# 4paradigm/OpenEmbedding

Measured on AMD Instinct MI355X. Metric: samples/sec DeepFM Criteo, higher is better.
Workload: dtype bf16; 1 GPU; model=deepfm-dim9, global_batch=4096, fields=26, dense_features=13, optimizer=adagrad, graph=True, prefetch=False, table=array, cache_mb=0, parallelism=single-gpu

## Files before the change

### openembedding_amd/ops/csrc/bindings.cpp

```cpp

#include <torch/extension.h>
#include <ATen/cuda/CUDAContext.h>
#include <c10/cuda/CUDAGuard.h>

#include <cstdint>
#include <tuple>
#include <vector>

typedef unsigned long long u64;
typedef int64_t i64;
typedef struct ihipStream_t* hipStream_t_;

extern "C" {
void emb_unique(const i64*, long, u64*, int*, long, int*, unsigned char*,
                i64*, i64*, int*, const i64*, int, hipStream_t_);
void emb_ht_lookup(u64*, int*, long, const i64*, long, int*, i64*, i64*,
                   unsigned char*, int, const int*, long, hipStream_t_);
void emb_ht_rehash(const u64*, const int*, long, u64*, int*, long,
                   hipStream_t_);
void emb_array_touch(unsigned char*, const i64*, long, long, long, i64*,
                     unsigned char*, const int*, hipStream_t_);
void emb_gather_init(float*, float*, long, long, const i64*,
                     const unsigned char*, const i64*, long, const i64*,
                     float*, int, float, float, float, u64, const float*,
                     const int*, hipStream_t_);
void emb_reduce_by_inverse(const i64*, const float*, long, long, float*, u64*,
                           long, hipStream_t_);
void emb_reduce_bags_by_inverse(const i64*, const float*, long, long,
                                const int*, const i64*, long, int, float*,
                                u64*, long, hipStream_t_);
void emb_pool_fwd(const float*, long, long, const i64*, long, const void*,
                  int, long, const i64*, long, int, float*, int*,
                  hipStream_t_);
void emb_pool_fwd_weighted(const float*, long, long, const i64*, long,
                           const void*, int, long, const i64*, long, int,
                           const float*, float*, int*, float*, hipStream_t_);
void emb_reduce_bags_weighted_by_inverse(const i64*, const float*, long, long,
                                         const int*, const float*,
// ... 77 lines not shown
using OptTensor = c10::optional<torch::Tensor>;

hipStream_t_ cur_stream() {
    return reinterpret_cast<hipStream_t_>(
        at::cuda::getCurrentCUDAStream().stream());
}

long next_pow2(long x) {
    long p = 16;
    while (p < x) p <<= 1;
    return p;
}

const int* u_ptr(const OptTensor& u_dev) {
    if (!u_dev.has_value()) return nullptr;
    TORCH_CHECK(u_dev->dtype() == torch::kInt32, "u_dev must be int32");
    return u_dev->data_ptr<int>();
}

#define CHECK_GPU(t) TORCH_CHECK((t).is_cuda(), #t " must be on GPU")
#define CHECK_CONT(t) TORCH_CHECK((t).is_contiguous(), #t " must be contiguous")


std::tuple<torch::Tensor, torch::Tensor, torch::Tensor> unique_bounded(
    torch::Tensor keys, OptTensor field_offsets) {
    CHECK_GPU(keys); CHECK_CONT(keys);
    TORCH_CHECK(keys.dtype() == torch::kInt64);
    const i64* foff = nullptr;
    int F = 0;
    if (field_offsets.has_value() && field_offsets->numel()) {
        CHECK_GPU(*field_offsets); CHECK_CONT(*field_offsets);
        TORCH_CHECK(field_offsets->dtype() == torch::kInt64,
                    "field_offsets must be int64");
        TORCH_CHECK(keys.numel() % field_offsets->numel() == 0,
                    "keys length must be a multiple of field_offsets");
        foff = field_offsets->data_ptr<i64>();
        F = (int)field_offsets->numel();
    }
    const c10::cuda::CUDAGuard guard(keys.device());
    long n = keys.numel();
    auto opts_i64 = keys.options();
    auto opts_i32 = keys.options().dtype(torch::kInt32);
    auto opts_u8 = keys.options().dtype(torch::kUInt8);
    long cap = next_pow2(2 * n);
    auto tk = torch::empty({cap}, opts_i64);
    auto tv = torch::empty({cap}, opts_i32);
    auto slot_of = torch::empty({n}, opts_i32);
    auto is_first = torch::empty({n}, opts_u8);
    auto uk = torch::empty({n}, opts_i64);
    auto inverse = torch::empty({n}, opts_i64);
    auto counter = torch::empty({1}, opts_i32);
    emb_unique(keys.data_ptr<i64>(), n, (u64*)tk.data_ptr<i64>(),
               tv.data_ptr<int>(), cap, slot_of.data_ptr<int>(),
               is_first.data_ptr<uint8_t>(), uk.data_ptr<i64>(),
               inverse.data_ptr<i64>(), counter.data_ptr<int>(), foff, F,
               cur_stream());
    return {uk, inverse, counter};
}

std::tuple<torch::Tensor, torch::Tensor> unique_inverse(torch::Tensor keys) {
    auto r = unique_bounded(keys, c10::nullopt);
    long u = std::get<2>(r).item<int>();
    return {std::get<0>(r).narrow(0, 0, u), std::get<1>(r)};
}


std::tuple<torch::Tensor, torch::Tensor> ht_lookup(
    torch::Tensor tk, torch::Tensor tv, torch::Tensor keys,
    torch::Tensor nrows, torch::Tensor slot_keys, bool insert,
    OptTensor u_dev) {
    CHECK_GPU(keys); CHECK_CONT(keys);
    const c10::cuda::CUDAGuard guard(keys.device());
    long n = keys.numel();
    auto slots = torch::empty({n}, keys.options());
    auto new_mask = torch::empty({n}, keys.options().dtype(torch::kUInt8));
    if (n)
        emb_ht_lookup((u64*)tk.data_ptr<i64>(), tv.data_ptr<int>(),
                      tk.numel(), keys.data_ptr<i64>(), n,
                      nrows.data_ptr<int>(), slot_keys.data_ptr<i64>(),
                      slots.data_ptr<i64>(), new_mask.data_ptr<uint8_t>(),
// ... 54 lines not shown
                    keys.data_ptr<i64>(), n,
                    inverse.has_value() ? inverse->data_ptr<i64>() : nullptr,
                    out_ptr, (int)init_cat,
                    (float)p0, (float)p1, (float)p2, (u64)seed,
                    sd ? state_init_row.data_ptr<float>() : nullptr,
                    u_ptr(u_dev), cur_stream());
    return out;
}


std::tuple<torch::Tensor, torch::Tensor> reduce_by_inverse(
    torch::Tensor inverse, torch::Tensor grads, int64_t u) {
    CHECK_GPU(grads); CHECK_CONT(grads);
    TORCH_CHECK(grads.dtype() == torch::kFloat32,
                "reduce_by_inverse: grads must be float32");
    const c10::cuda::CUDAGuard guard(grads.device());
    long n = grads.size(0);
    long dim = grads.size(1);
    auto ugrads = torch::empty({u, dim}, grads.options());
    auto counts = torch::empty({u}, grads.options().dtype(torch::kInt64));
    emb_reduce_by_inverse(inverse.data_ptr<i64>(), grads.data_ptr<float>(), n,
                          dim, ugrads.data_ptr<float>(),
                          (u64*)counts.data_ptr<i64>(), u, cur_stream());
    return {ugrads, counts};
}


std::tuple<torch::Tensor, torch::Tensor> pool_fwd(
    torch::Tensor rows, OptTensor inverse, OptTensor map,
    torch::Tensor offsets, int64_t mode, bool want_bag_of) {
    CHECK_GPU(rows); CHECK_CONT(rows);
    CHECK_GPU(offsets); CHECK_CONT(offsets);
    TORCH_CHECK(rows.dtype() == torch::kFloat32 && rows.dim() == 2,
                "pool_fwd: rows must be float32 [R, dim]");
    TORCH_CHECK(offsets.dtype() == torch::kInt64 && offsets.dim() == 1
                && offsets.numel() >= 1,
                "pool_fwd: offsets must be int64 [B+1]");
    TORCH_CHECK(mode >= 0 && mode <= 2, "pool_fwd: bad mode");
    const void* map_ptr = nullptr;
    int map_kind = 0;
    long u = 0;
    if (map.has_value()) {
        CHECK_GPU(*map); CHECK_CONT(*map);
        u = map->numel();
        if (map->dtype() == torch::kInt64) {
            map_kind = 1;
// ... 846 lines not shown
                 w2t.data_ptr(), w1t.data_ptr(), H, Hp, dz1.data_ptr(),
                 dz2.data_ptr(), dz3.data_ptr(), dx0.data_ptr(), bptr,
                 (int)bm, (int)frag, cur_stream());
    return {dx0, dz1, dz2, dz3};
}

}

PYBIND11_MODULE(TORCH_EXTENSION_NAME, m) {
    m.def("unique_inverse", &unique_inverse, "hash-based unique+inverse");
    m.def("unique_bounded", &unique_bounded,
          "unique+inverse without host sync (n-sized buffer + device "
          "count); optional fused per-field key offsets",
          pybind11::arg("keys"),
          pybind11::arg("field_offsets") = pybind11::none());
    m.def("ht_lookup", &ht_lookup, "hash table lookup/insert");
    m.def("ht_rehash", &ht_rehash, "hash table rehash into larger table");
    m.def("array_touch", &array_touch,
          "array-table slot compute + valid-bitmap touch");
    m.def("gather_init", &gather_init,
          "row gather with fused lazy init (+ optional duplicate scatter)");
    m.def("reduce_by_inverse", &reduce_by_inverse,
          "grad reduce-by-key with counts (LDS-aggregated)");
    m.def("pool_fwd", &pool_fwd,
          "segment-pooled gather (sum/mean/sqrtn) over ragged bags; also "
          "emits each element's bag for the backward",
          pybind11::arg("rows"), pybind11::arg("inverse"),
          pybind11::arg("map"), pybind11::arg("offsets"),
          pybind11::arg("mode"), pybind11::arg("want_bag_of") = true);
    m.def("reduce_bags_by_inverse", &reduce_bags_by_inverse,
          "grad reduce-by-key reading the pooled [B, dim] gradient through "
          "bag_of (no [nnz, dim] expansion)");
    m.def("pool_fwd_weighted", &pool_fwd_weighted,
          "pool_fwd with per-sample weights; also emits bag_of and the "
          "per-bag combiner scale for the backward",
          pybind11::arg("rows"), pybind11::arg("inverse"),
          pybind11::arg("map"), pybind11::arg("offsets"),
          pybind11::arg("weights"), pybind11::arg("mode"),
          pybind11::arg("out") = pybind11::none(),
          pybind11::arg("bag_scale") = pybind11::none());
    m.def("reduce_bags_weighted_by_inverse",
          &reduce_bags_weighted_by_inverse,
          "bag-indirected grad reduce with the per-element factor "
          "weights[e] * bag_scale[bag_of[e]]");
    m.def("pool_wgrad", &pool_wgrad,
          "gradient of the weighted pool w.r.t. its per-sample weights",
// ... 97 lines not shown
```

### openembedding_amd/ops/csrc/embops.hip

```cpp

#include <hip/hip_runtime.h>
#include <cstdint>

#define DEV static __device__ __forceinline__

typedef unsigned long long u64;
typedef long long i64;

static constexpr u64 EMPTY = ~0ull;
static constexpr int BLOCK = 256;

static inline int cdiv(long a, long b) { return (int)((a + b - 1) / b); }
static inline int grid1d(long n) {
    long g = (n + BLOCK - 1) / BLOCK;
    return (int)(g < 1 ? 1 : g);
}


template <typename T>
__global__ void k_fill(T* __restrict__ p, long n, T v) {
    long i = (long)blockIdx.x * blockDim.x + threadIdx.x;
    if (i < n) p[i] = v;
}

static inline void fill_u64(u64* p, long n, u64 v, hipStream_t s) {
    if (n) k_fill<u64><<<(int)((n + 255) / 256), 256, 0, s>>>(p, n, v);
}
static inline void fill_i32(int* p, long n, int v, hipStream_t s) {
    if (n) k_fill<int><<<(int)((n + 255) / 256), 256, 0, s>>>(p, n, v);
}
static inline void fill_u8(unsigned char* p, long n, unsigned char v,
                           hipStream_t s) {
    if (n) k_fill<unsigned char><<<(int)((n + 255) / 256), 256, 0, s>>>(p, n, v);
}
static inline void fill_f32(float* p, long n, float v, hipStream_t s) {
    if (n) k_fill<float><<<(int)((n + 255) / 256), 256, 0, s>>>(p, n, v);
}

__global__ void k_unique_reset(u64* __restrict__ tk, long cap,
                               unsigned char* __restrict__ is_first, long n,
                               int* __restrict__ counter) {
    long i = (long)blockIdx.x * blockDim.x + threadIdx.x;
    if (i < cap) tk[i] = ~0ull;
    if (i < n) is_first[i] = 0;
    if (i == 0) *counter = 0;
}

__global__ void k_reduce_reset(float* __restrict__ ugrads, long ne,
                               u64* __restrict__ counts, long u) {
    long i = (long)blockIdx.x * blockDim.x + threadIdx.x;
    if (i < ne) ugrads[i] = 0.0f;
    if (i < u) counts[i] = 0ull;
}

__global__ void k_pad_reset(u64* __restrict__ send_keys,
                            int* __restrict__ send_src, long total,
                            int* __restrict__ counts, long world) {
    long i = (long)blockIdx.x * blockDim.x + threadIdx.x;
    if (i < total) { send_keys[i] = ~0ull; send_src[i] = -1; }
    if (i < world) counts[i] = 0;
}


DEV u64 splitmix64(u64 z) {
    z += 0x9E3779B97F4A7C15ull;
    z = (z ^ (z >> 30)) * 0xBF58476D1CE4E5B9ull;
    z = (z ^ (z >> 27)) * 0x94D049BB133111EBull;
    return z ^ (z >> 31);
// ... 17 lines not shown
    float r = sqrtf(-2.0f * logf(1.0f - u1));
    return r * cosf(2.0f * 3.14159265358979323846f * u2);
}

DEV float init_value(int cat, float p0, float p1, float p2,
                     u64 seed, u64 key, u64 col) {
    if (cat == INIT_CONSTANT) return p0;
    if (cat == INIT_UNIFORM) {
        float u = uniform01(seed, key, col, 0);
        return p0 + u * p1;
    }
    float z = normal01(seed, key, col, 0);
    if (p2 > 0.1f) {
        for (int attempt = 1; attempt < 16 && z > p2; ++attempt)
            z = normal01(seed, key, col, attempt);
    }
    return p0 + p1 * z;
}


#define ULDS 1024
#define UA_ITERS 8
#define UI_ILP 4

__global__ void k_unique_insert(const i64* __restrict__ keys, long n,
                                u64* __restrict__ tk, long mask,
                                int* __restrict__ slot_of,
                                unsigned char* __restrict__ is_first,
                                const i64* __restrict__ foff, int F) {
    __shared__ u64 lkeys[ULDS];
    __shared__ int lslot[ULDS];
    for (int t = threadIdx.x; t < ULDS; t += blockDim.x) lkeys[t] = EMPTY;
    __syncthreads();

    long i = (long)blockIdx.x * blockDim.x + threadIdx.x;
    u64 k = 0;
    i64 kin = 0;
    if (i < n) {
        kin = keys[i];
        if (foff) kin += foff[(int)i % F];
    }
    int lh = -1;
    bool lds_winner = false, lds_ok = false;
    if (i < n && (u64)kin == EMPTY) {
        is_first[i] = 1;
        slot_of[i] = -1;
    } else if (i < n) {
        k = (u64)kin;
        u64 hh = splitmix64(k);
        lh = (int)(hh & (ULDS - 1));
        for (int probes = 0; probes < 64; ++probes) {
            u64 cur = atomicCAS(&lkeys[lh], EMPTY, k);
            if (cur == EMPTY) { lds_winner = true; lds_ok = true; break; }
            if (cur == k) { lds_ok = true; break; }
            lh = (lh + 1) & (ULDS - 1);
        }
        if (lds_winner || !lds_ok) {
            u64 h = splitmix64(k) & (u64)mask;
            long found = -1;
            for (long p = 0; p <= mask; ++p) {
                u64 cur = tk[h];
                if (cur == k) { found = (long)h; break; }
                if (cur == EMPTY) {
                    u64 prev = atomicCAS(&tk[h], EMPTY, k);
                    if (prev == EMPTY) {
                        is_first[i] = 1; found = (long)h; break;
                    }
                    if (prev == k) { found = (long)h; break; }
                }
                h = (h + 1) & (u64)mask;
            }
            if (found < 0) is_first[i] = 1;
            slot_of[i] = found >= 0 ? (int)found : -1;
            if (lds_winner)
                lslot[lh] = found >= 0 ? (int)found : (int)(-2 - i);
        }
    }
    __syncthreads();
    if (i < n && lds_ok && !lds_winner) slot_of[i] = lslot[lh];
}

__global__ void k_unique_assign(const i64* __restrict__ keys, long n,
                                const int* __restrict__ slot_of,
                                const unsigned char* __restrict__ is_first,
                                int* __restrict__ tv,
                                i64* __restrict__ unique_keys,
                                int* __restrict__ counter,
                                i64* __restrict__ inverse,
                                const i64* __restrict__ foff, int F) {
    const int lane = threadIdx.x & 63;
    const long stride = (long)gridDim.x * blockDim.x;
    long i0 = (long)blockIdx.x * blockDim.x + threadIdx.x;
    u64 ballots[UA_ITERS];
    int total = 0;
    #pragma unroll
    for (int t = 0; t < UA_ITERS; ++t) {
        long i = i0 + t * stride;
        bool first = (i < n) && is_first[i];
        ballots[t] = __ballot(first);
        total += __popcll(ballots[t]);
    }
    if (!total) return;
    int base = 0;
    if (lane == 0) base = atomicAdd(counter, total);
    base = __shfl(base, 0, 64);
    #pragma unroll
    for (int t = 0; t < UA_ITERS; ++t) {
        u64 b = ballots[t];
        if (b & (1ull << lane)) {
            long i = i0 + t * stride;
            int uid = base + __popcll(b & ((1ull << lane) - 1ull));
            i64 kin = keys[i];
            if (foff) kin += foff[(int)i % F];
            unique_keys[uid] = kin;
            int s = slot_of[i];
            if (s >= 0) tv[s] = uid;
            else inverse[i] = uid;
        }
        base += __popcll(b);
    }
}

__global__ void k_unique_inverse(long n, const int* __restrict__ slot_of,
                                 const int* __restrict__ tv,
                                 i64* __restrict__ inverse) {
    const long stride = (long)gridDim.x * blockDim.x;
    long i0 = (long)blockIdx.x * blockDim.x + threadIdx.x;
    int s[UI_ILP];
    #pragma unroll
    for (int t = 0; t < UI_ILP; ++t) {
        long i = i0 + t * stride;
        s[t] = (i < n) ? slot_of[i] : -1;
    }
    int v[UI_ILP];
    #pragma unroll
    for (int t = 0; t < UI_ILP; ++t)
        v[t] = (s[t] >= 0) ? tv[s[t]] : 0;
    #pragma unroll
    for (int t = 0; t < UI_ILP; ++t) {
        long i = i0 + t * stride;
        if (i >= n) continue;
        if (s[t] >= 0) inverse[i] = (i64)v[t];
        else if (s[t] <= -2) inverse[i] = inverse[-2 - s[t]];
    }
}


__global__ void k_ht_lookup(u64* __restrict__ tk, int* __restrict__ tv,
                            long mask, const i64* __restrict__ keys, long n,
                            int* __restrict__ nrows,
                            i64* __restrict__ slot_keys,
                            i64* __restrict__ slots,
                            unsigned char* __restrict__ new_mask,
                            int insert, const int* __restrict__ u_dev,
                            long row_cap) {
    long i = (long)blockIdx.x * blockDim.x + threadIdx.x;
    if (i >= n) return;
    if (u_dev && i >= *u_dev) {
        slots[i] = -1;
        if (new_mask) new_mask[i] = 0;
        return;
    }
    u64 k = (u64)keys[i];
    if (k == EMPTY) {
// ... 493 lines not shown
        long src;
        if constexpr (WEIGHTED)
            src = reduce_src_w(bag_of[i], B, weights[i], bag_scale, scale);
        else
            src = reduce_src(bag_of[i], n, offsets, B, mode, scale);
        if (src < 0) return;
        atomicAdd(&ugrads[inverse[i] * dim + j],
                  grads[(u64)src * dim + j] * scale);
    } else {
        atomicAdd(&ugrads[inverse[i] * dim + j], grads[e]);
    }
}

template <bool BAG = false>
__global__ void k_reduce_counts(const i64* __restrict__ inverse, long n,
                                u64* __restrict__ counts,
                                const int* __restrict__ bag_of, long B) {
    long i = (long)blockIdx.x * blockDim.x + threadIdx.x;
    if (i >= n) return;
    if (BAG && (bag_of[i] < 0 || bag_of[i] >= B)) return;
    atomicAdd(&counts[inverse[i]], 1ull);
}

#define WG_ILP 4
template <int G, typename MapT>
__global__ void k_pool_wgrad(const float* __restrict__ rows, long R,
                             long dim, const i64* __restrict__ inverse,
                             long nnz, const MapT* __restrict__ map, long u,
                             const float* __restrict__ weights,
                             const int* __restrict__ bag_of,
                             const float* __restrict__ bag_scale,
                             const float* __restrict__ out,
                             const float* __restrict__ grad_out, long B,
                             int mode, float* __restrict__ dw) {
    const long e = ((long)blockIdx.x * blockDim.x + threadIdx.x) / G;
    const int lane = threadIdx.x % G;
    if (e >= nnz) return;
    const int bag = bag_of[e];
    if (bag < 0 || bag >= B) {
        if (lane == 0) dw[e] = 0.0f;
        return;
    }
    const long nidx = map ? u : R;
    const long row = pool_row(e, nnz, inverse, map, nidx, R);
    const float scale = bag_scale[bag];
    const float* __restrict__ g = grad_out + (u64)bag * dim;
// ... 563 lines not shown
    else LAUNCH_POOL(64, 4, 4);
#undef LAUNCH_POOL
}

template <bool WEIGHTED, typename Resolve>
static void pool_lookup_dispatch(const float* rows, long dim, long nnz,
                                 const i64* offsets, long B, int mode,
                                 const float* weights, float* out,
                                 const Resolve& resolve,
                                 hipStream_t stream) {
    if (B == 0) return;
#define LAUNCH_LOOKUP(G, CF, ILP)                                           \
    k_pool_lookup<G, CF, ILP, WEIGHTED, Resolve>                            \
        <<<grid1d(B * G), BLOCK, 0, stream>>>(rows, dim, nnz, offsets, B,   \
                                              mode, weights, out, resolve)
    if (dim <= 16) LAUNCH_LOOKUP(16, 1, 16);
    else if (dim <= 32) LAUNCH_LOOKUP(16, 2, 8);
    else if (dim <= 64) LAUNCH_LOOKUP(64, 1, 16);
    else if (dim <= 128) LAUNCH_LOOKUP(64, 2, 8);
    else LAUNCH_LOOKUP(64, 4, 4);
#undef LAUNCH_LOOKUP
}

extern "C" {

void emb_unique(const i64* keys, long n, u64* tk, int* tv, long cap,
                int* slot_of, unsigned char* is_first, i64* unique_keys,
                i64* inverse, int* counter, const i64* foff, int F,
                hipStream_t stream) {
    {
        long mx = cap > n ? cap : n;
        k_unique_reset<<<(int)((mx + 255) / 256), 256, 0, stream>>>(
            tk, cap, is_first, n, counter);
    }
    long mask = cap - 1;
    k_unique_insert<<<grid1d(n), BLOCK, 0, stream>>>(keys, n, tk, mask,
                                                     slot_of, is_first,
                                                     foff, F);
    int ga = grid1d((n + UA_ITERS - 1) / UA_ITERS);
    int gi = grid1d((n + UI_ILP - 1) / UI_ILP);
    k_unique_assign<<<ga, BLOCK, 0, stream>>>(keys, n, slot_of, is_first,
                                              tv, unique_keys, counter,
                                              inverse, foff, F);
    k_unique_inverse<<<gi, BLOCK, 0, stream>>>(n, slot_of, tv, inverse);
}

void emb_ht_lookup(u64* tk, int* tv, long cap, const i64* keys, long n,
                   int* nrows, i64* slot_keys, i64* slots,
                   unsigned char* new_mask, int insert, const int* u_dev,
                   long row_cap, hipStream_t stream) {
    k_ht_lookup<<<grid1d(n), BLOCK, 0, stream>>>(tk, tv, cap - 1, keys, n,
                                                 nrows, slot_keys, slots,
                                                 new_mask, insert, u_dev,
                                                 row_cap);
}

void emb_ht_rehash(const u64* tk_old, const int* tv_old, long cap_old,
                   u64* tk_new, int* tv_new, long cap_new,
                   hipStream_t stream) {
    fill_u64(tk_new, cap_new, EMPTY, stream);
    k_ht_rehash<<<grid1d(cap_old), BLOCK, 0, stream>>>(
        tk_old, tv_old, cap_old, tk_new, tv_new, cap_new - 1);
}

void emb_array_touch(unsigned char* valid, const i64* keys, long n,
                     long shard_num, long cap, i64* slots,
                     unsigned char* new_mask, const int* u_dev,
// ... 314 lines not shown
```

### openembedding_amd/ops/dispatch.py

```python

from __future__ import annotations

from typing import Tuple

import torch

from . import require_hip


def _use_hip(t: torch.Tensor) -> bool:
    return t.is_cuda



def unique_inverse(keys: torch.Tensor) -> Tuple[torch.Tensor, torch.Tensor]:
    if keys.numel() == 0:
        return keys.clone(), torch.empty(0, dtype=torch.int64, device=keys.device)
    if _use_hip(keys):
        ext = require_hip()
        if ext is not None:
            return ext.unique_inverse(keys)
    return torch.unique(keys, return_inverse=True)



def reduce_by_inverse(inverse: torch.Tensor, grads: torch.Tensor, u: int
                      ) -> Tuple[torch.Tensor, torch.Tensor]:
    if _use_hip(grads) and grads.dtype == torch.float32:
        ext = require_hip()
        if ext is not None:
            return ext.reduce_by_inverse(inverse, grads, u)
    ugrads = torch.zeros((u, grads.shape[1]), dtype=grads.dtype,
                         device=grads.device)
    ugrads.index_add_(0, inverse, grads)
    counts = torch.bincount(inverse, minlength=u).to(torch.int64)
    return ugrads, counts



POOL_MODES = {"sum": 0, "mean": 1, "sqrtn": 2}


def _bag_scale(offsets: torch.Tensor, nnz: int, mode: str,
               dtype: torch.dtype) -> torch.Tensor:
    off = offsets.clamp(0, nnz)
    length = (off[1:] - off[:-1]).clamp(min=0).to(dtype)
    if mode == "sum":
        scale = torch.ones_like(length)
    elif mode == "mean":
        scale = 1.0 / length
    else:
        scale = 1.0 / length.sqrt()
    return torch.where(length > 0, scale, torch.zeros_like(scale))


def _bag_of(offsets: torch.Tensor, nnz: int) -> torch.Tensor:
    off = offsets.clamp(0, nnz)
    pos = torch.arange(nnz, device=offsets.device)
# ... 205 lines not shown
```

### openembedding_amd/parallel/sharded.py

```python

from __future__ import annotations

import dataclasses
import os
from typing import Dict, List, Optional

import torch

from ..core.variable import VariableShard
from ..ops import dispatch as ops
from ..utils.metrics import REGISTRY, stage_timer
from . import comm


class _PaddedPlan:

    def __init__(self, world: int, n: int, device: torch.device):
        slack = float(os.environ.get("OEAMD_A2A_SLACK", "2.0"))
        cap = int(-(-n * slack // world))
        cap = (cap + 255) // 256 * 256
        self.cap = max(1, min(n, cap))
        self.world = world
        total = world * self.cap
        self.send_keys = torch.full((total,), -1, dtype=torch.int64,
                                    device=device)
        self.send_src = torch.full((total,), -1, dtype=torch.int32,
                                   device=device)
        self.pos_of = torch.full((n,), -1, dtype=torch.int32, device=device)
        self.counts = torch.zeros(world, dtype=torch.int32, device=device)
        self.overflow = torch.zeros(1, dtype=torch.int32, device=device)
        self.overflow_host = 0


@dataclasses.dataclass
class PullHandle:

    shape: torch.Size
    unique: Optional[torch.Tensor] = None
    inverse: Optional[torch.Tensor] = None
    order: Optional[torch.Tensor] = None
    send_splits: Optional[List[int]] = None
    recv_splits: Optional[List[int]] = None
    owner_unique: Optional[torch.Tensor] = None
    owner_inverse: Optional[torch.Tensor] = None
    bounded: bool = False
    u_dev: Optional[torch.Tensor] = None
    slots: Optional[torch.Tensor] = None
    owner_u_dev: Optional[torch.Tensor] = None
    owner_slots: Optional[torch.Tensor] = None
    padded: bool = False
    plan: Optional["_PaddedPlan"] = None
    owner_cpu: Optional[tuple] = None
    bag_of: Optional[torch.Tensor] = None
    bag_scale: Optional[torch.Tensor] = None
    pooled_rows: Optional[torch.Tensor] = None


class ShardedVariable:

    def __init__(self, shard: VariableShard, storage=None):
        self.shard = shard
        self.storage = storage
        self.world_size = shard.shard_num
        self.rank = shard.shard_id
        self.stat_pull_indices = 0
        self.stat_pull_unique = 0
        self._plans: Dict[int, Optional[_PaddedPlan]] = {}
        self._commits_since_check = 0


    @property
    def meta(self):
        return self.shard.meta

    @property
    def variable_id(self):
        return self.shard.meta.variable_id

# ... 34 lines not shown
                r = self._pull_remote_padded(indices, flat, field_offsets)
                if r is not None:
                    return r
            if bounded_ok:
                return self._pull_remote_bounded(indices, flat,
                                                 field_offsets)
        unique, inverse = ops.unique_inverse(flat)
        self.stat_pull_unique += unique.numel()
        REGISTRY.add("pull_indices", n)
        REGISTRY.add("pull_unique", unique.numel())
        h = PullHandle(shape=indices.shape, unique=unique, inverse=inverse)
        if self.world_size == 1:
            rows_u = (self.shard.pull_readonly(unique) if readonly
                      else self.shard.pull(unique))
        else:
            rows_u = self._pull_remote(h, readonly)
        out = rows_u.index_select(0, inverse)
        out = out.view(*h.shape, self.shard.dim)
        return out, h

    def _pull_local_bounded(self, indices: torch.Tensor, flat: torch.Tensor,
                            field_offsets: torch.Tensor = None):
        ext = self.shard.ext
        uk_buf, inverse, u_dev = ext.unique_bounded(flat, field_offsets)
        out, slots = self.shard.pull_bounded(uk_buf, u_dev, inverse)
        h = PullHandle(shape=indices.shape, unique=uk_buf, inverse=inverse,
                       bounded=True, u_dev=u_dev, slots=slots)
        return out.view(*indices.shape, self.shard.dim), h

    def pull_pooled(self, values: torch.Tensor, offsets: torch.Tensor,
                    mode: str, readonly: bool = False, pre=None,
                    weights: torch.Tensor = None, wgrad: bool = False):
        flat = values.reshape(-1).to(torch.int64)
        dim = self.shard.dim
        gpu = getattr(self.shard, "pull_bounded", None) is not None
        remote = self.world_size > 1 or self._force_remote
        if gpu and not remote and not readonly and pre is None:
            self.stat_pull_indices += flat.numel()
            ext = self.shard.ext
            uk_buf, inverse, u_dev = ext.unique_bounded(flat, None)
            bag_scale = None
            if weights is None:
                out, slots, bag_of = self.shard.pull_pooled_bounded(
                    uk_buf, u_dev, inverse, offsets, ops.POOL_MODES[mode])
            else:
                out, slots, bag_of, bag_scale = \
                    self.shard.pull_pooled_bounded(
                        uk_buf, u_dev, inverse, offsets,
                        ops.POOL_MODES[mode], weights)
            h = PullHandle(shape=flat.shape, unique=uk_buf, inverse=inverse,
# ... 91 lines not shown
                dev = device if comm.backend() == "nccl" else "cpu"
                t = torch.tensor([n, -n], dtype=torch.int64, device=dev)
                dist.all_reduce(t, op=dist.ReduceOp.MIN)
                if int(t[0]) != n or int(-t[1]) != n:
                    self._plans[n] = None
                    return None
            pair = [_PaddedPlan(self.world_size, n, device),
                    _PaddedPlan(self.world_size, n, device), 0]
            self._plans[n] = pair
        pair[2] ^= 1
        return pair[pair[2]]

    def _pull_remote_padded(self, indices: torch.Tensor,
                            flat: torch.Tensor,
                            field_offsets: torch.Tensor = None):
        world = self.world_size
        dim = self.shard.dim
        dev = flat.device
        n = flat.numel()
        plan = self._get_padded_plan(n, dev)
        if plan is None:
            return None
        gpu = getattr(self.shard, "pull_bounded", None) is not None
        if gpu:
            ext = self.shard.ext
            uk_buf, inverse, u_dev = ext.unique_bounded(flat, field_offsets)
            ext.bucketize_pad(uk_buf, u_dev, world, plan.cap,
                              plan.send_keys, plan.send_src, plan.pos_of,
                              plan.counts, plan.overflow)
        else:
            uk_buf, inverse = ops.unique_inverse(flat)
            u_dev = None
            self._bucketize_pad_torch(uk_buf, plan)
        REGISTRY.add("pull_indices", n)
        REGISTRY.add("pull_wire_keys", plan.send_keys.numel())
        h = PullHandle(shape=indices.shape, unique=uk_buf, inverse=inverse,
                       u_dev=u_dev, padded=True, plan=plan)
        recv_keys = comm.all_to_all_equal(plan.send_keys, world)
        if gpu:
            uk2_buf, inv2, u2_dev = ext.unique_bounded(recv_keys)
            rows_back, slots2 = self.shard.pull_bounded(uk2_buf, u2_dev,
                                                        inv2)
            h.owner_unique = uk2_buf
            h.owner_inverse = inv2
            h.owner_u_dev = u2_dev
            h.owner_slots = slots2
        else:
            rows_back = self._owner_pull_padded_torch(recv_keys, h)
        rows_recv = comm.all_to_all_equal(rows_back, world)
        if gpu:
            out = ext.scatter_out(rows_recv, inverse, plan.pos_of, n)
        else:
            pos = plan.pos_of.index_select(0, inverse).long()
            out = rows_recv.index_select(0, pos.clamp(min=0))
            out = out.masked_fill((pos < 0).unsqueeze(1), 0.0)
        return out.view(*indices.shape, dim), h

    def _bucketize_pad_torch(self, uk: torch.Tensor,
                             plan: _PaddedPlan) -> None:
        world, cap = plan.world, plan.cap
# ... 98 lines not shown
            h.owner_unique = uk2_buf
            h.owner_inverse = inv2
            h.owner_u_dev = u2_dev
            h.owner_slots = slots2
        else:
            uk2, inv2 = ops.unique_inverse(recv_keys)
            rows_u2 = (self.shard.pull_readonly(uk2) if readonly
                       else self.shard.pull(uk2))
            rows_back = rows_u2.index_select(0, inv2)
            h.owner_unique = uk2
            h.owner_inverse = inv2
        rows_sorted = comm.all_to_all_v(rows_back, recv_splits, send_splits)
        rows_u = torch.empty_like(rows_sorted)
        rows_u.index_copy_(0, order, rows_sorted)
        h.order = order
        h.send_splits = send_splits
        h.recv_splits = recv_splits
        return rows_u


    def push(self, h: PullHandle, grads: torch.Tensor) -> None:
        dim = self.shard.dim
        g = grads.reshape(-1, dim)
        ugrads, counts = ops.reduce_by_inverse(h.inverse, g,
                                               h.unique.numel())
        self._apply_reduced(h, ugrads, counts)

    def push_pooled(self, h: PullHandle, grad_out: torch.Tensor,
                    offsets: torch.Tensor, mode: str,
                    weights: torch.Tensor = None, out: torch.Tensor = None,
                    wgrad: bool = False):
        g = grad_out.reshape(-1, self.shard.dim)
        if weights is None:
            ugrads, counts = ops.reduce_bags_by_inverse(
                h.inverse, g, h.bag_of, offsets, mode, h.unique.numel())
            self._apply_reduced(h, ugrads, counts)
            return None
        nnz = h.bag_of.numel()
        w = weights[:nnz].contiguous()
        ugrads, counts = ops.reduce_bags_weighted_by_inverse(
            h.inverse, g, h.bag_of, w, h.bag_scale, h.unique.numel())
        dw = None
        if wgrad:
            if h.pooled_rows is not None:
                dw = ops.pool_wgrad(h.pooled_rows, None, None, w, h.bag_of,
                                    h.bag_scale, out, g, mode)
                h.pooled_rows = None
            else:
# ... 57 lines not shown
```

Baseline: 17.52 million samples/s.

## Build inverted index during unique and reduce gradients by segment without atomics

The unique kernels now also count occurrences per slot, compute per-uid segment offsets with a wave prefix scan, and write a permutation that groups each unique key's occurrences. This gives an inverted index. A new segmented reduce kernel walks each uid's list to sum gradients and set counts, which replaces the atomic reduce-by-inverse in push. Lists longer than a threshold are handled by dedicated blocks. The cost is extra atomics, memory traffic and bookkeeping inside unique, and it is on by default through an environment flag.

```diff
diff --git a/openembedding_amd/ops/csrc/bindings.cpp b/openembedding_amd/ops/csrc/bindings.cpp
--- a/openembedding_amd/ops/csrc/bindings.cpp
+++ b/openembedding_amd/ops/csrc/bindings.cpp
@@ -14,6 +14,15 @@
 extern "C" {
 void emb_unique(const i64*, long, u64*, int*, long, int*, unsigned char*,
                 i64*, i64*, int*, const i64*, int, hipStream_t_);
+void emb_unique_indexed(const i64*, long, u64*, int*, long, int*,
+                        unsigned char*, i64*, i64*, int*, const i64*, int,
+                        int*, int*, int*, int*, int*, int*, int*, long, int*,
+                        int*, hipStream_t_);
+int emb_seg_threshold();
+int emb_seg_max_dim();
+void emb_reduce_by_index(const int*, const int*, const int*, const int*,
+                         const int*, long, const float*, long, long,
+                         const int*, float*, u64*, hipStream_t_);
 void emb_ht_lookup(u64*, int*, long, const i64*, long, int*, i64*, i64*,
                    unsigned char*, int, const int*, long, hipStream_t_);
 void emb_ht_rehash(const u64*, const int*, long, u64*, int*, long,
@@ -137,8 +146,8 @@
 #define CHECK_CONT(t) TORCH_CHECK((t).is_contiguous(), #t " must be contiguous")
 
 
-std::tuple<torch::Tensor, torch::Tensor, torch::Tensor> unique_bounded(
-    torch::Tensor keys, OptTensor field_offsets) {
+std::vector<torch::Tensor> unique_bounded_impl(
+    torch::Tensor keys, OptTensor field_offsets, bool indexed) {
     CHECK_GPU(keys); CHECK_CONT(keys);
     TORCH_CHECK(keys.dtype() == torch::kInt64);
     const i64* foff = nullptr;
@@ -165,12 +174,47 @@
     auto uk = torch::empty({n}, opts_i64);
     auto inverse = torch::empty({n}, opts_i64);
     auto counter = torch::empty({1}, opts_i32);
-    emb_unique(keys.data_ptr<i64>(), n, (u64*)tk.data_ptr<i64>(),
-               tv.data_ptr<int>(), cap, slot_of.data_ptr<int>(),
-               is_first.data_ptr<uint8_t>(), uk.data_ptr<i64>(),
-               inverse.data_ptr<i64>(), counter.data_ptr<int>(), foff, F,
-               cur_stream());
-    return {uk, inverse, counter};
+    if (!indexed) {
+        emb_unique(keys.data_ptr<i64>(), n, (u64*)tk.data_ptr<i64>(),
+                   tv.data_ptr<int>(), cap, slot_of.data_ptr<int>(),
+                   is_first.data_ptr<uint8_t>(), uk.data_ptr<i64>(),
+                   inverse.data_ptr<i64>(), counter.data_ptr<int>(), foff, F,
+                   cur_stream());
+        return {uk, inverse, counter};
+    }
+    TORCH_CHECK(n < (1L << 31), "unique_bounded_indexed: n must fit int32");
+    auto tct = torch::empty({2, cap}, opts_i32);
+    auto segs = torch::empty({4, n}, opts_i32);
+    long long_cap = n / (emb_seg_threshold() + 1) + 1;
+    auto long_list = torch::empty({long_cap}, opts_i32);
+    auto ctr = torch::empty({32}, opts_i32);
+    auto seg_off = segs.select(0, 0), seg_cnt = segs.select(0, 1);
+    auto perm = segs.select(0, 2), rank = segs.select(0, 3);
+    auto n_long = ctr.narrow(0, 16, 1);
+    emb_unique_indexed(keys.data_ptr<i64>(), n, (u64*)tk.data_ptr<i64>(),
+                       tv.data_ptr<int>(), cap, slot_of.data_ptr<int>(),
+                       is_first.data_ptr<uint8_t>(), uk.data_ptr<i64>(),
+                       inverse.data_ptr<i64>(), counter.data_ptr<int>(), foff,
+                       F, tct.data_ptr<int>(), tct.data_ptr<int>() + cap,
+                       rank.data_ptr<int>(), seg_off.data_ptr<int>(),
+                       seg_cnt.data_ptr<int>(), perm.data_ptr<int>(),
+                       long_list.data_ptr<int>(), long_cap,
+                       ctr.data_ptr<int>(), n_long.data_ptr<int>(),
+                       cur_stream());
+    return {uk, inverse, counter, seg_off, seg_cnt, perm, long_list, n_long};
+}
+
+std::tuple<torch::Tensor, torch::Tensor, torch::Tensor> unique_bounded(
+    torch::Tensor keys, OptTensor field_offsets) {
+    auto r = unique_bounded_impl(keys, field_offsets, false);
+    return {r[0], r[1], r[2]};
+}
+
+std::tuple<torch::Tensor, torch::Tensor, torch::Tensor, torch::Tensor,
+           torch::Tensor, torch::Tensor, torch::Tensor, torch::Tensor>
+unique_bounded_indexed(torch::Tensor keys, OptTensor field_offsets) {
+    auto r = unique_bounded_impl(keys, field_offsets, true);
+    return {r[0], r[1], r[2], r[3], r[4], r[5], r[6], r[7]};
 }
 
 std::tuple<torch::Tensor, torch::Tensor> unique_inverse(torch::Tensor keys) {
@@ -271,6 +315,39 @@
     emb_reduce_by_inverse(inverse.data_ptr<i64>(), grads.data_ptr<float>(), n,
                           dim, ugrads.data_ptr<float>(),
                           (u64*)counts.data_ptr<i64>(), u, cur_stream());
+    return {ugrads, counts};
+}
+
+std::tuple<torch::Tensor, torch::Tensor> reduce_by_index(
+    torch::Tensor seg_off, torch::Tensor seg_cnt, torch::Tensor perm,
+    torch::Tensor long_list, torch::Tensor n_long, torch::Tensor grads,
+    torch::Tensor u_dev) {
+    CHECK_GPU(grads); CHECK_CONT(grads);
+    TORCH_CHECK(grads.dtype() == torch::kFloat32 && grads.dim() == 2,
+                "reduce_by_index: grads must be float32 [n, dim]");
+    long n = grads.size(0);
+    long dim = grads.size(1);
+    TORCH_CHECK(dim <= emb_seg_max_dim(),
+                "reduce_by_index: dim above the kernel's ladder");
+    for (const auto* t : {&seg_off, &seg_cnt, &perm, &long_list, &n_long,
+                          &u_dev}) {
+        CHECK_GPU(*t); CHECK_CONT(*t);
+        TORCH_CHECK(t->dtype() == torch::kInt32,
+                    "reduce_by_index: index tensors must be int32");
+    }
+    TORCH_CHECK(seg_off.numel() == n && seg_cnt.numel() == n
+                && perm.numel() == n,
+                "reduce_by_index: index does not match grads");
+    TORCH_CHECK(n_long.numel() == 1 && u_dev.numel() == 1);
+    const c10::cuda::CUDAGuard guard(grads.device());
+    auto ugrads = torch::empty({n, dim}, grads.options());
+    auto counts = torch::empty({n}, grads.options().dtype(torch::kInt64));
+    emb_reduce_by_index(seg_off.data_ptr<int>(), seg_cnt.data_ptr<int>(),
+                        perm.data_ptr<int>(), long_list.data_ptr<int>(),
+                        n_long.data_ptr<int>(), long_list.numel(),
+                        grads.data_ptr<float>(), n, dim,
+                        u_dev.data_ptr<int>(), ugrads.data_ptr<float>(),
+                        (u64*)counts.data_ptr<i64>(), cur_stream());
     return {ugrads, counts};
 }
 
@@ -1163,6 +1240,18 @@
           "row gather with fused lazy init (+ optional duplicate scatter)");
     m.def("reduce_by_inverse", &reduce_by_inverse,
           "grad reduce-by-key with counts (LDS-aggregated)");
+    m.def("unique_bounded_indexed", &unique_bounded_indexed,
+          "unique_bounded plus the batch's inverted index (seg_off, "
+          "seg_cnt, perm, long_list, n_long)",
+          pybind11::arg("keys"),
+          pybind11::arg("field_offsets") = pybind11::none());
+    m.def("reduce_by_index", &reduce_by_index,
+          "grad reduce-by-key with counts through the inverted index "
+          "(segmented, no atomics)");
+    m.def("seg_reduce_threshold", &emb_seg_threshold,
+          "list length above which a uid is in long_list");
+    m.def("seg_reduce_max_dim", &emb_seg_max_dim,
+          "widest dim reduce_by_index covers");
     m.def("pool_fwd", &pool_fwd,
           "segment-pooled gather (sum/mean/sqrtn) over ragged bags; also "
           "emits each element's bag for the backward",
diff --git a/openembedding_amd/ops/csrc/embops.hip b/openembedding_amd/ops/csrc/embops.hip
--- a/openembedding_amd/ops/csrc/embops.hip
+++ b/openembedding_amd/ops/csrc/embops.hip
@@ -37,13 +37,33 @@
     if (n) k_fill<float><<<(int)((n + 255) / 256), 256, 0, s>>>(p, n, v);
 }
 
+struct UIdx {
+    int* tcount;
+    int* toff;
+    int* rank;
+    int* seg_off;
+    int* seg_cnt;
+    int* perm;
+    int* long_list;
+    int* off_counter;
+    int* n_long;
+    long long_cap;
+};
+
+template <bool IDX>
 __global__ void k_unique_reset(u64* __restrict__ tk, long cap,
                                unsigned char* __restrict__ is_first, long n,
-                               int* __restrict__ counter) {
+                               int* __restrict__ counter, UIdx ix) {
     long i = (long)blockIdx.x * blockDim.x + threadIdx.x;
-    if (i < cap) tk[i] = ~0ull;
+    if (i < cap) {
+        tk[i] = ~0ull;
+        if constexpr (IDX) ix.tcount[i] = 0;
+    }
     if (i < n) is_first[i] = 0;
-    if (i == 0) *counter = 0;
+    if (i == 0) {
+        *counter = 0;
+        if constexpr (IDX) { *ix.off_counter = 0; *ix.n_long = 0; }
+    }
 }
 
 __global__ void k_reduce_reset(float* __restrict__ ugrads, long ne,
@@ -107,15 +127,23 @@
 #define ULDS 1024
 #define UA_ITERS 8
 #define UI_ILP 4
-
+#define SEG_T 32
+
+template <bool IDX>
 __global__ void k_unique_insert(const i64* __restrict__ keys, long n,
                                 u64* __restrict__ tk, long mask,
                                 int* __restrict__ slot_of,
                                 unsigned char* __restrict__ is_first,
-                                const i64* __restrict__ foff, int F) {
+                                const i64* __restrict__ foff, int F,
+                                UIdx ix) {
     __shared__ u64 lkeys[ULDS];
     __shared__ int lslot[ULDS];
-    for (int t = threadIdx.x; t < ULDS; t += blockDim.x) lkeys[t] = EMPTY;
+    __shared__ int lcnt[IDX ? ULDS : 1];
+    __shared__ int lbase[IDX ? ULDS : 1];
+    for (int t = threadIdx.x; t < ULDS; t += blockDim.x) {
+        lkeys[t] = EMPTY;
+        if constexpr (IDX) lcnt[t] = 0;
+    }
     __syncthreads();
 
     long i = (long)blockIdx.x * blockDim.x + threadIdx.x;
@@ -126,6 +154,7 @@
         if (foff) kin += foff[(int)i % F];
     }
     int lh = -1;
+    int lr = 0;
     bool lds_winner = false, lds_ok = false;
     if (i < n && (u64)kin == EMPTY) {
         is_first[i] = 1;
@@ -140,6 +169,8 @@
             if (cur == k) { lds_ok = true; break; }
             lh = (lh + 1) & (ULDS - 1);
         }
+        if constexpr (IDX)
+            if (lds_ok) lr = atomicAdd(&lcnt[lh], 1);
         if (lds_winner || !lds_ok) {
             u64 h = splitmix64(k) & (u64)mask;
             long found = -1;
@@ -159,12 +190,24 @@
             slot_of[i] = found >= 0 ? (int)found : -1;
             if (lds_winner)
                 lslot[lh] = found >= 0 ? (int)found : (int)(-2 - i);
+            if constexpr (IDX)
+                if (!lds_ok && found >= 0)
+                    lr = atomicAdd(&ix.tcount[found], 1);
         }
     }
     __syncthreads();
     if (i < n && lds_ok && !lds_winner) slot_of[i] = lslot[lh];
-}
-
+    if constexpr (IDX) {
+        if (lds_winner) {
+            int s = lslot[lh];
+            lbase[lh] = s >= 0 ? atomicAdd(&ix.tcount[s], lcnt[lh]) : 0;
+        }
+        __syncthreads();
+        if (i < n) ix.rank[i] = lds_ok ? lbase[lh] + lr : lr;
+    }
+}
+
+template <bool IDX>
 __global__ void k_unique_assign(const i64* __restrict__ keys, long n,
                                 const int* __restrict__ slot_of,
                                 const unsigned char* __restrict__ is_first,
@@ -172,23 +215,48 @@
                                 i64* __restrict__ unique_keys,
                                 int* __restrict__ counter,
                                 i64* __restrict__ inverse,
-                                const i64* __restrict__ foff, int F) {
+                                const i64* __restrict__ foff, int F,
+                                UIdx ix) {
     const int lane = threadIdx.x & 63;
     const long stride = (long)gridDim.x * blockDim.x;
     long i0 = (long)blockIdx.x * blockDim.x + threadIdx.x;
     u64 ballots[UA_ITERS];
+    int sl[IDX ? UA_ITERS : 1], c[IDX ? UA_ITERS : 1];
     int total = 0;
     #pragma unroll
     for (int t = 0; t < UA_ITERS; ++t) {
         long i = i0 + t * stride;
+        if constexpr (IDX) sl[t] = (i < n) ? slot_of[i] : -1;
         bool first = (i < n) && is_first[i];
         ballots[t] = __ballot(first);
         total += __popcll(ballots[t]);
     }
     if (!total) return;
-    int base = 0;
-    if (lane == 0) base = atomicAdd(counter, total);
+    int off = 0, wtot = 0;
+    if constexpr (IDX) {
+        int ctot = 0;
+        #pragma unroll
+        for (int t = 0; t < UA_ITERS; ++t) {
+            c[t] = (ballots[t] >> lane & 1ull)
+                       ? (sl[t] >= 0 ? ix.tcount[sl[t]] : 1) : 0;
+            ctot += c[t];
+        }
+        int inc = ctot;
+        #pragma unroll
+        for (int d = 1; d < 64; d <<= 1) {
+            int v = __shfl_up(inc, d, 64);
+            if (lane >= d) inc += v;
+        }
+        wtot = __shfl(inc, 63, 64);
+        off = inc - ctot;
+    }
+    int base = 0, obase = 0;
+    if (lane == 0) {
+        base = atomicAdd(counter, total);
+        if constexpr (IDX) obase = atomicAdd(ix.off_counter, wtot);
+    }
     base = __shfl(base, 0, 64);
+    if constexpr (IDX) off += __shfl(obase, 0, 64);
     #pragma unroll
     for (int t = 0; t < UA_ITERS; ++t) {
         u64 b = ballots[t];
@@ -198,17 +266,30 @@
             i64 kin = keys[i];
             if (foff) kin += foff[(int)i % F];
             unique_keys[uid] = kin;
-            int s = slot_of[i];
+            int s;
+            if constexpr (IDX) s = sl[t]; else s = slot_of[i];
             if (s >= 0) tv[s] = uid;
             else inverse[i] = uid;
+            if constexpr (IDX) {
+                ix.seg_off[uid] = off;
+                ix.seg_cnt[uid] = c[t];
+                if (s >= 0) ix.toff[s] = off;
+                else if (off >= 0 && off < n) ix.perm[off] = (int)i;
+                if (c[t] > SEG_T) {
+                    int q = atomicAdd(ix.n_long, 1);
+                    if (q < ix.long_cap) ix.long_list[q] = uid;
+                }
+                off += c[t];
+            }
         }
         base += __popcll(b);
     }
 }
 
+template <bool IDX>
 __global__ void k_unique_inverse(long n, const int* __restrict__ slot_of,
                                  const int* __restrict__ tv,
-                                 i64* __restrict__ inverse) {
+                                 i64* __restrict__ inverse, UIdx ix) {
     const long stride = (long)gridDim.x * blockDim.x;
     long i0 = (long)blockIdx.x * blockDim.x + threadIdx.x;
     int s[UI_ILP];
@@ -218,13 +299,23 @@
         s[t] = (i < n) ? slot_of[i] : -1;
     }
     int v[UI_ILP];
+    int r[IDX ? UI_ILP : 1], o[IDX ? UI_ILP : 1];
     #pragma unroll
-    for (int t = 0; t < UI_ILP; ++t)
+    for (int t = 0; t < UI_ILP; ++t) {
         v[t] = (s[t] >= 0) ? tv[s[t]] : 0;
+        if constexpr (IDX) {
+            o[t] = (s[t] >= 0) ? ix.toff[s[t]] : 0;
+            r[t] = (s[t] >= 0) ? ix.rank[i0 + t * stride] : 0;
+        }
+    }
     #pragma unroll
     for (int t = 0; t < UI_ILP; ++t) {
         long i = i0 + t * stride;
         if (i >= n) continue;
+        if constexpr (IDX) {
+            long p = (long)o[t] + r[t];
+            if (s[t] >= 0 && p >= 0 && p < n) ix.perm[p] = (int)i;
+        }
         if (s[t] >= 0) inverse[i] = (i64)v[t];
         else if (s[t] <= -2) inverse[i] = inverse[-2 - s[t]];
     }
@@ -764,6 +855,155 @@
     atomicAdd(&counts[inverse[i]], 1ull);
 }
 
+#define SR_ILP 4
+#define LR_ILP 8
+#define SEG_BLOCK 1024
+#define SEG_LONG_BLOCKS 256
+#define SEG_MAX_DIM 128
+
+DEV void seg_range(const int* __restrict__ seg_off,
+                   const int* __restrict__ seg_cnt, long uid, long n,
+                   int& off, int& cnt) {
+    int o = seg_off[uid], c = seg_cnt[uid];
+    o = o < 0 ? 0 : (o > n ? (int)n : o);
+    c = c < 0 ? 0 : c;
+    off = o;
+    cnt = c > n - o ? (int)(n - o) : c;
+}
+
+template <int G, int CF>
+__global__ __launch_bounds__(SEG_BLOCK)
+void k_seg_reduce(const int* __restrict__ seg_off,
+                  const int* __restrict__ seg_cnt,
+                  const int* __restrict__ perm,
+                  const int* __restrict__ long_list,
+                  const int* __restrict__ n_long, long long_cap,
+                  int long_blocks, const float* __restrict__ grads, long n,
+                  long dim, const int* __restrict__ u_dev,
+                  float* __restrict__ ugrads, u64* __restrict__ counts) {
+    __shared__ float red[SEG_BLOCK / 64][G * CF];
+    const int lane = threadIdx.x % G;
+    long u = *u_dev;
+    u = u < 0 ? 0 : (u > n ? n : u);
+
+    if ((int)blockIdx.x < long_blocks) {
+        long nl = *n_long;
+        nl = nl < 0 ? 0 : (nl > long_cap ? long_cap : nl);
+        const int group = threadIdx.x / G;
+        constexpr int NG = SEG_BLOCK / G;
+        for (long b = blockIdx.x; b < nl; b += long_blocks) {
+            const int uid = long_list[b];
+            int off = 0, cnt = 0;
+            if (uid >= 0 && uid < u)
+                seg_range(seg_off, seg_cnt, uid, n, off, cnt);
+            if (cnt <= SEG_T) continue;
+            float acc[CF];
+            #pragma unroll
+            for (int c = 0; c < CF; ++c) acc[c] = 0.0f;
+            int e[LR_ILP], en[LR_ILP];
+            #pragma unroll
+            for (int t = 0; t < LR_ILP; ++t)
+                en[t] = (group * LR_ILP + t < cnt)
+                            ? perm[off + group * LR_ILP + t] : -1;
+            for (long base = group * LR_ILP; base < cnt;
+                 base += NG * LR_ILP) {
+                #pragma unroll
+                for (int t = 0; t < LR_ILP; ++t) {
+                    e[t] = (en[t] < 0 || en[t] >= n) ? -1 : en[t];
+                    const long nx = base + NG * LR_ILP + t;
+                    en[t] = (nx < cnt) ? perm[off + nx] : -1;
+                }
+                float v[LR_ILP][CF];
+                #pragma unroll
+                for (int t = 0; t < LR_ILP; ++t)
+                    #pragma unroll
+                    for (int c = 0; c < CF; ++c)
+                        v[t][c] = (e[t] >= 0 && lane + c * G < dim)
+                            ? grads[(u64)e[t] * dim + lane + c * G] : 0.0f;
+                #pragma unroll
+                for (int t = 0; t < LR_ILP; ++t)
+                    #pragma unroll
+                    for (int c = 0; c < CF; ++c) acc[c] += v[t][c];
+            }
+            #pragma unroll
+            for (int d = G; d < 64; d <<= 1)
+                #pragma unroll
+                for (int c = 0; c < CF; ++c)
+                    acc[c] += __shfl_xor(acc[c], d, 64);
+            if ((threadIdx.x & 63) < G) {
+                #pragma unroll
+                for (int c = 0; c < CF; ++c)
+                    red[threadIdx.x / 64][lane + c * G] = acc[c];
+            }
+            __syncthreads();
+            if (threadIdx.x < G * CF) {
+                float s = 0.0f;
+                #pragma unroll
+                for (int w = 0; w < SEG_BLOCK / 64; ++w)
+                    s += red[w][threadIdx.x];
+                if (threadIdx.x < dim)
+                    ugrads[(u64)uid * dim + threadIdx.x] = s;
+            }
+            if (threadIdx.x == 0) counts[uid] = (u64)cnt;
+            __syncthreads();
+        }
+        return;
+    }
+
+    const long ngroups = (long)(gridDim.x - long_blocks) * (SEG_BLOCK / G);
+    const long g0 = ((long)(blockIdx.x - long_blocks) * SEG_BLOCK
+                     + threadIdx.x) / G;
+    int off[SR_ILP], cnt[SR_ILP], e0[SR_ILP];
+    #pragma unroll
+    for (int t = 0; t < SR_ILP; ++t) {
+        long uid = g0 + t * ngroups;
+        off[t] = 0;
+        cnt[t] = 0;
+        if (uid < u) seg_range(seg_off, seg_cnt, uid, n, off[t], cnt[t]);
+    }
+    #pragma unroll
+    for (int t = 0; t < SR_ILP; ++t) {
+        e0[t] = (cnt[t] > 0 && cnt[t] <= SEG_T) ? perm[off[t]] : -1;
+        if (e0[t] < 0 || e0[t] >= n) e0[t] = -1;
+    }
+    float acc[SR_ILP][CF];
+    #pragma unroll
+    for (int t = 0; t < SR_ILP; ++t)
+        #pragma unroll
+        for (int c = 0; c < CF; ++c)
+            acc[t][c] = (e0[t] >= 0 && lane + c * G < dim)
+                ? grads[(u64)e0[t] * dim + lane + c * G] : 0.0f;
+    #pragma unroll
+    for (int t = 0; t < SR_ILP; ++t) {
+        long uid = g0 + t * ngroups;
+        if (uid >= n || cnt[t] > SEG_T) continue;
+        for (int k = 1; k < cnt[t]; k += SR_ILP) {
+            int e[SR_ILP];
+            #pragma unroll
+            for (int q = 0; q < SR_ILP; ++q) {
+                e[q] = (k + q < cnt[t]) ? perm[off[t] + k + q] : -1;
+                if (e[q] < 0 || e[q] >= n) e[q] = -1;
+            }
+            float v[SR_ILP][CF];
+            #pragma unroll
+            for (int q = 0; q < SR_ILP; ++q)
+                #pragma unroll
+                for (int c = 0; c < CF; ++c)
+                    v[q][c] = (e[q] >= 0 && lane + c * G < dim)
+                        ? grads[(u64)e[q] * dim + lane + c * G] : 0.0f;
+            #pragma unroll
+            for (int q = 0; q < SR_ILP; ++q)
+                #pragma unroll
+                for (int c = 0; c < CF; ++c) acc[t][c] += v[q][c];
+        }
+        #pragma unroll
+        for (int c = 0; c < CF; ++c)
+            if (lane + c * G < dim)
+                ugrads[(u64)uid * dim + lane + c * G] = acc[t][c];
+        if (lane == 0) counts[uid] = (u64)cnt[t];
+    }
+}
+
 #define WG_ILP 4
 template <int G, typename MapT>
 __global__ void k_pool_wgrad(const float* __restrict__ rows, long R,
@@ -1373,27 +1613,75 @@
 #undef LAUNCH_LOOKUP
 }
 
+template <bool IDX>
+static void unique_launch(const i64* keys, long n, u64* tk, int* tv, long cap,
+                          int* slot_of, unsigned char* is_first,
+                          i64* unique_keys, i64* inverse, int* counter,
+                          const i64* foff, int F, const UIdx& ix,
+                          hipStream_t stream) {
+    {
+        long mx = cap > n ? cap : n;
+        k_unique_reset<IDX><<<(int)((mx + 255) / 256), 256, 0, stream>>>(
+            tk, cap, is_first, n, counter, ix);
+    }
+    long mask = cap - 1;
+    k_unique_insert<IDX><<<grid1d(n), BLOCK, 0, stream>>>(
+        keys, n, tk, mask, slot_of, is_first, foff, F, ix);
+    int ga = grid1d((n + UA_ITERS - 1) / UA_ITERS);
+    int gi = grid1d((n + UI_ILP - 1) / UI_ILP);
+    k_unique_assign<IDX><<<ga, BLOCK, 0, stream>>>(
+        keys, n, slot_of, is_first, tv, unique_keys, counter, inverse, foff,
+        F, ix);
+    k_unique_inverse<IDX><<<gi, BLOCK, 0, stream>>>(n, slot_of, tv, inverse,
+                                                    ix);
+}
+
 extern "C" {
 
 void emb_unique(const i64* keys, long n, u64* tk, int* tv, long cap,
                 int* slot_of, unsigned char* is_first, i64* unique_keys,
                 i64* inverse, int* counter, const i64* foff, int F,
                 hipStream_t stream) {
-    {
-        long mx = cap > n ? cap : n;
-        k_unique_reset<<<(int)((mx + 255) / 256), 256, 0, stream>>>(
-            tk, cap, is_first, n, counter);
-    }
-    long mask = cap - 1;
-    k_unique_insert<<<grid1d(n), BLOCK, 0, stream>>>(keys, n, tk, mask,
-                                                     slot_of, is_first,
-                                                     foff, F);
-    int ga = grid1d((n + UA_ITERS - 1) / UA_ITERS);
-    int gi = grid1d((n + UI_ILP - 1) / UI_ILP);
-    k_unique_assign<<<ga, BLOCK, 0, stream>>>(keys, n, slot_of, is_first,
-                                              tv, unique_keys, counter,
-                                              inverse, foff, F);
-    k_unique_inverse<<<gi, BLOCK, 0, stream>>>(n, slot_of, tv, inverse);
+    unique_launch<false>(keys, n, tk, tv, cap, slot_of, is_first,
+                         unique_keys, inverse, counter, foff, F, UIdx{},
+                         stream);
+}
+
+void emb_unique_indexed(const i64* keys, long n, u64* tk, int* tv, long cap,
+                        int* slot_of, unsigned char* is_first,
+                        i64* unique_keys, i64* inverse, int* counter,
+                        const i64* foff, int F, int* tcount, int* toff,
+                        int* rank, int* seg_off, int* seg_cnt, int* perm,
+                        int* long_list, long long_cap, int* off_counter,
+                        int* n_long, hipStream_t stream) {
+    UIdx ix{tcount, toff, rank, seg_off, seg_cnt, perm, long_list,
+            off_counter, n_long, long_cap};
+    unique_launch<true>(keys, n, tk, tv, cap, slot_of, is_first, unique_keys,
+                        inverse, counter, foff, F, ix, stream);
+}
+
+int emb_seg_threshold() { return SEG_T; }
+int emb_seg_max_dim() { return SEG_MAX_DIM; }
+
+void emb_reduce_by_index(const int* seg_off, const int* seg_cnt,
+                         const int* perm, const int* long_list,
+                         const int* n_long, long long_cap,
+                         const float* grads, long n, long dim,
+                         const int* u_dev, float* ugrads, u64* counts,
+                         hipStream_t stream) {
+    if (n == 0) return;
+    int lb = (int)(long_cap < SEG_LONG_BLOCKS ? long_cap : SEG_LONG_BLOCKS);
+    long groups = (n + SR_ILP - 1) / SR_ILP;
+#define LAUNCH_SEG(G, CF)                                                   \
+    k_seg_reduce<G, CF>                                                     \
+        <<<lb + cdiv(groups * G, SEG_BLOCK), SEG_BLOCK, 0, stream>>>(       \
+            seg_off, seg_cnt, perm, long_list, n_long, long_cap, lb, grads, \
+            n, dim, u_dev, ugrads, counts)
+    if (dim <= 16) LAUNCH_SEG(16, 1);
+    else if (dim <= 32) LAUNCH_SEG(16, 2);
+    else if (dim <= 64) LAUNCH_SEG(64, 1);
+    else LAUNCH_SEG(64, 2);
+#undef LAUNCH_SEG
 }
 
 void emb_ht_lookup(u64* tk, int* tv, long cap, const i64* keys, long n,
diff --git a/openembedding_amd/ops/dispatch.py b/openembedding_amd/ops/dispatch.py
--- a/openembedding_amd/ops/dispatch.py
+++ b/openembedding_amd/ops/dispatch.py
@@ -34,6 +34,36 @@
                          device=grads.device)
     ugrads.index_add_(0, inverse, grads)
     counts = torch.bincount(inverse, minlength=u).to(torch.int64)
+    return ugrads, counts
+
+
+def seg_reduce_covers(grads: torch.Tensor) -> bool:
+    if not (_use_hip(grads) and grads.dtype == torch.float32):
+        return False
+    ext = require_hip()
+    return ext is not None and grads.shape[1] <= ext.seg_reduce_max_dim()
+
+
+def reduce_by_index(index, grads: torch.Tensor, u_dev
+                    ) -> Tuple[torch.Tensor, torch.Tensor]:
+    seg_off, seg_cnt, perm, long_list, n_long = index
+    if seg_reduce_covers(grads):
+        return require_hip().reduce_by_index(seg_off, seg_cnt, perm,
+                                             long_list, n_long, grads, u_dev)
+    n = grads.shape[0]
+    u = int(u_dev)
+    dev = grads.device
+    cnt = seg_cnt[:u].to(dev, torch.int64)
+    start = seg_off[:u].to(dev, torch.int64)
+    uid = torch.repeat_interleave(torch.arange(u, device=dev), cnt)
+    first = torch.cumsum(cnt, 0) - cnt
+    pos = (torch.arange(uid.numel(), device=dev)
+           + torch.repeat_interleave(start - first, cnt))
+    elems = perm.to(dev, torch.int64).index_select(0, pos)
+    ugrads = torch.zeros((n, grads.shape[1]), dtype=grads.dtype, device=dev)
+    ugrads.index_add_(0, uid, grads.index_select(0, elems))
+    counts = torch.zeros(n, dtype=torch.int64, device=dev)
+    counts[:u] = cnt
     return ugrads, counts
 
 
diff --git a/openembedding_amd/parallel/sharded.py b/openembedding_amd/parallel/sharded.py
--- a/openembedding_amd/parallel/sharded.py
+++ b/openembedding_amd/parallel/sharded.py
@@ -11,6 +11,16 @@
 from ..ops import dispatch as ops
 from ..utils.metrics import REGISTRY, stage_timer
 from . import comm
+
+
+_SEG_REDUCE = os.environ.get("OEAMD_SEG_REDUCE", "1") != "0"
+
+
+def _unique_bounded(ext, flat: torch.Tensor, field_offsets):
+    if not _SEG_REDUCE:
+        return (*ext.unique_bounded(flat, field_offsets), None)
+    r = ext.unique_bounded_indexed(flat, field_offsets)
+    return r[0], r[1], r[2], tuple(r[3:])
 
 
 class _PaddedPlan:
@@ -54,6 +64,7 @@
     bag_of: Optional[torch.Tensor] = None
     bag_scale: Optional[torch.Tensor] = None
     pooled_rows: Optional[torch.Tensor] = None
+    index: Optional[tuple] = None
 
 
 class ShardedVariable:
@@ -134,10 +145,11 @@
     def _pull_local_bounded(self, indices: torch.Tensor, flat: torch.Tensor,
                             field_offsets: torch.Tensor = None):
         ext = self.shard.ext
-        uk_buf, inverse, u_dev = ext.unique_bounded(flat, field_offsets)
+        uk_buf, inverse, u_dev, index = _unique_bounded(ext, flat,
+                                                        field_offsets)
         out, slots = self.shard.pull_bounded(uk_buf, u_dev, inverse)
         h = PullHandle(shape=indices.shape, unique=uk_buf, inverse=inverse,
-                       bounded=True, u_dev=u_dev, slots=slots)
+                       bounded=True, u_dev=u_dev, slots=slots, index=index)
         return out.view(*indices.shape, self.shard.dim), h
 
     def pull_pooled(self, values: torch.Tensor, offsets: torch.Tensor,
@@ -275,9 +287,11 @@
         if plan is None:
             return None
         gpu = getattr(self.shard, "pull_bounded", None) is not None
+        index = None
         if gpu:
             ext = self.shard.ext
-            uk_buf, inverse, u_dev = ext.unique_bounded(flat, field_offsets)
+            uk_buf, inverse, u_dev, index = _unique_bounded(ext, flat,
+                                                            field_offsets)
             ext.bucketize_pad(uk_buf, u_dev, world, plan.cap,
                               plan.send_keys, plan.send_src, plan.pos_of,
                               plan.counts, plan.overflow)
@@ -288,7 +302,7 @@
         REGISTRY.add("pull_indices", n)
         REGISTRY.add("pull_wire_keys", plan.send_keys.numel())
         h = PullHandle(shape=indices.shape, unique=uk_buf, inverse=inverse,
-                       u_dev=u_dev, padded=True, plan=plan)
+                       u_dev=u_dev, padded=True, plan=plan, index=index)
         recv_keys = comm.all_to_all_equal(plan.send_keys, world)
         if gpu:
             uk2_buf, inv2, u2_dev = ext.unique_bounded(recv_keys)
@@ -433,8 +447,11 @@
     def push(self, h: PullHandle, grads: torch.Tensor) -> None:
         dim = self.shard.dim
         g = grads.reshape(-1, dim)
-        ugrads, counts = ops.reduce_by_inverse(h.inverse, g,
-                                               h.unique.numel())
+        if h.index is not None and ops.seg_reduce_covers(g):
+            ugrads, counts = ops.reduce_by_index(h.index, g, h.u_dev)
+        else:
+            ugrads, counts = ops.reduce_by_inverse(h.inverse, g,
+                                                   h.unique.numel())
         self._apply_reduced(h, ugrads, counts)
 
     def push_pooled(self, h: PullHandle, grad_out: torch.Tensor,
```

Result: faster. 19.16 million samples/s, median of 6 (+9.4%).
